# minaskar/pocomc

Measured on AMD Instinct MI355X. Metric: preconditioned MCMC steps/sec (1e4 particles, 32-D), higher is better.
Workload: dtype f32 flow (MFMA) + f64 step

## Files before the change

include/pocomc_amd.h:

```cpp
#ifndef POCOMC_AMD_H
#define POCOMC_AMD_H

#include <stdint.h>

#ifdef __cplusplus
extern "C" {
#endif

#define PMC_ABI_VERSION 9

const char* pmc_last_error(void);
int pmc_abi_version(void);
const char* pmc_build_id(void);


typedef struct pmc_maf {
    const float* packed;
    const int32_t* meta;
    int32_t D, H, T;
    int32_t Hp, Dp;
    int32_t nT, nXT, nOT;
    int64_t pk_per_transform;
    int32_t tri_ok;
    int32_t n_out;
// ... 366 lines not shown
    const pmc_prior_stage_t* prior_stage;
} pmc_step_ext_t;

int pmc_blob_rows_move(const int32_t* accept, const void* src, void* dst, int64_t n, int64_t row_bytes, void* stream);

#define PMC_ADAPT_TPCN 1
#define PMC_ADAPT_PRWM 2
#define PMC_ADAPT_RWM 3
#define PMC_ADAPT_MU 8

int pmc_rng_fill(const pmc_rng_t* rng, double gamma_shape, double* normal, double* gamma, double* uniform,
                 int64_t n, int32_t D, void* stream);
int pmc_event_synchronize(void* ev);

int pmc_propose_inverse(int kind, const float* cur32, const double* mu, const double* inv_cov, const double* chol,
                        double nu, double sigma, double cn_a, const pmc_rng_t* rng, double* prop64, double* quad,
                        double* quad_prop, const pmc_maf_t* maf, float* u_out, float* ladj, int64_t n, void* stream);

int pmc_step_pre(const pmc_step_t* s, const pmc_rng_t* rng, double nu, double sigma, double cn_a, void* stream);
int pmc_step_pre_deferred(const pmc_step_t* s, const pmc_rng_t* rng, double nu, double sigma, double cn_a, void* stream);
int pmc_step_fill_next(const pmc_step_t* s, const pmc_rng_t* rng, double nu, void* stream);
int pmc_step_handover(const pmc_step_t* s, int64_t step, int32_t epilogue, pmc_handover_t* out, int32_t* mode,
                      int32_t* clean_unknown);
int pmc_step_post(const pmc_step_t* s, const pmc_rng_t* rng, double beta, double nu, int want_mask,
                  int copy_sums, void* stream);
int pmc_step_lik_rows(const pmc_step_t* s, void* stream);
int pmc_step_prior_rows(const pmc_step_t* s, const void* logp, int logp_is_f32, void* stream);
int pmc_step_prior_stage(const pmc_step_t* s, void* stream);
int pmc_adapt_update(const double* const* parts, int32_t n_parts, int32_t D, double* total_out, double* h_sums,
                     double* adapt_state, int32_t adapt_mode, double c_sigma, double c_mu, double cap, double n_total,
                     const pmc_done_t* done, void* stream);
int pmc_stream_synchronize(void* stream);

void* pmc_comm_create(int32_t rank, int32_t world, int32_t width);
void* pmc_comm_create_host(int32_t rank, int32_t world, int32_t width);
int pmc_comm_kind(void* comm);
int pmc_comm_unlink(void* comm);
int pmc_comm_handle(void* comm, void* out64);
int pmc_comm_connect(void* comm, const void* handles);
void pmc_comm_destroy(void* comm);
int pmc_comm_adapt_update(void* comm, const double* const* parts, int32_t n_parts, int32_t D, double* total_out, double* h_sums,
                          double* adapt_state, int32_t adapt_mode, double c_sigma, double c_mu, double cap, double n_total,
                          const pmc_done_t* done, double timeout_s, void* stream);
int pmc_pipeline_set_comm(void* pipeline, void* comm);

void* pmc_pipeline_create(const pmc_step_t* const* lanes, int32_t n_lanes, uint64_t seed, const uint64_t* offsets,
                          void* prefetcher, double wait_timeout_s, void* stream);
void pmc_pipeline_destroy(void* pipeline);
int pmc_pipeline_start(void* pipeline, double nu, int64_t first_step);
int pmc_pipeline_next(void* pipeline, int32_t lane_done, double beta, double nu, int32_t adapt_mode, double c_sigma,
                      double c_mu, double cap, double n_total, int32_t more);
int pmc_pipeline_stats(void* pipeline, double* out, int32_t reset);
void* pmc_event_create(void);
int pmc_event_record(void* ev, void* stream);
float pmc_event_elapsed_ms(void* a, void* b);
void pmc_event_destroy(void* ev);


int pmc_logw(const double* logl, const double* beta, const double* logz, double beta_final,
             double* logw, int32_t T, int64_t N, void* stream);

int64_t pmc_reduce_workspace_bytes(int64_t P);
int pmc_logw_stats(const double* logw, int64_t P, int64_t k, double* stats, void* workspace, void* stream);

int64_t pmc_trim_workspace_bytes(int64_t P);
int pmc_trim_threshold(const double* w, int64_t P, double ess, int32_t bins, double* result,
                       void* workspace, int64_t workspace_bytes, void* stream);


int pmc_weights_from_logw(const double* logw, int64_t P, const double* stats, double* w, void* stream);

// ... 154 lines not shown
```

pocomc_amd/_lib.py:

```python
from __future__ import annotations

import ctypes as C
import os

_HERE = os.path.dirname(os.path.abspath(__file__))
LIB_PATH = os.environ.get("PMC_LIBRARY") or os.path.join(_HERE, "libpocomc_amd.so")

c_p = C.c_void_p


class pmc_maf_t(C.Structure):
    _fields_ = [("packed", c_p), ("meta", c_p),
                ("D", C.c_int32), ("H", C.c_int32), ("T", C.c_int32),
                ("Hp", C.c_int32), ("Dp", C.c_int32),
                ("nT", C.c_int32), ("nXT", C.c_int32), ("nOT", C.c_int32),
                ("pk_per_transform", C.c_int64),
                ("tri_ok", C.c_int32), ("n_out", C.c_int32),
                ("lane16", c_p), ("lane16_fmt", C.c_int32), ("reserved", C.c_int32)]


class pmc_inverse_plan_t(C.Structure):
    _fields_ = [(k, C.c_int32) for k in ("sweep", "fused", "epilogue", "maxo", "fm", "subsets", "waves", "helper_fmt",
                                         "lds_bytes")]

# ... 181 lines not shown
    "pmc_maf_valid_epoch": (C.c_int, [P(pmc_maf_t), c_p, c_p, c_p, i64, i64, c_p, c_p, c_p]),
    "pmc_neg_weighted_sum": (C.c_int, [c_p, c_p, c_p, C.c_float, c_p, i64, c_p]),
    "pmc_sum_f32": (C.c_int, [c_p, c_p, i64, c_p]),
    "pmc_adamw_step": (C.c_int, [c_p, c_p, c_p, c_p, i64, f64, f64, f64, f64, f64, f64, i64, c_p, c_p]),
    "pmc_scaler_inverse": (C.c_int, [P(pmc_scaler_t), c_p, c_p, c_p, c_p, c_p, c_p, c_p, i64, c_p]),
    "pmc_scaler_forward": (C.c_int, [P(pmc_scaler_t), c_p, c_p, i64, c_p]),
    "pmc_prior_logpdf": (C.c_int, [P(pmc_prior_t), c_p, c_p, c_p, i64, c_p]),
    "pmc_scaler_inverse_prior": (C.c_int, [P(pmc_scaler_t), P(pmc_prior_t), c_p, c_p, c_p, c_p, c_p, c_p, c_p, c_p,
                                           c_p, c_p, P(pmc_done_t), i64, c_p]),
    "pmc_wait_flag": (C.c_int, [c_p, i64, f64]),
    "pmc_propose": (C.c_int, [C.c_int, c_p, c_p, c_p, c_p, c_p, f64, f64, f64, P(pmc_rng_t),
                              c_p, c_p, c_p, c_p, i64, i32, c_p]),
    "pmc_accept_workspace_bytes": (i64, [i64, i32]),
    "pmc_accept": (C.c_int, [C.c_int, C.c_int, P(pmc_state_t), P(pmc_proposal_t), f64, f64,
                             P(pmc_rng_t), c_p, c_p, c_p, c_p, i64, i32, c_p]),
    "pmc_accept_armed": (C.c_int, [C.c_int, C.c_int, P(pmc_state_t), P(pmc_proposal_t), f64, f64,
                                   P(pmc_rng_t), c_p, c_p, c_p, c_p, P(pmc_done_t), c_p, i64, i32, c_p]),
    "pmc_propose_inverse": (C.c_int, [C.c_int, c_p, c_p, c_p, c_p, f64, f64, f64, P(pmc_rng_t), c_p, c_p, c_p,
                                      P(pmc_maf_t), c_p, c_p, i64, c_p]),
    "pmc_step_pre": (C.c_int, [P(pmc_step_t), P(pmc_rng_t), f64, f64, f64, c_p]),
    "pmc_step_pre_deferred": (C.c_int, [P(pmc_step_t), P(pmc_rng_t), f64, f64, f64, c_p]),
    "pmc_step_fill_next": (C.c_int, [P(pmc_step_t), P(pmc_rng_t), f64, c_p]),
    "pmc_step_handover": (C.c_int, [P(pmc_step_t), i64, i32, P(pmc_handover_t), P(i32), P(i32)]),
    "pmc_step_post": (C.c_int, [P(pmc_step_t), P(pmc_rng_t), f64, f64, C.c_int, C.c_int, c_p]),
    "pmc_step_lik_rows": (C.c_int, [P(pmc_step_t), c_p]),
    "pmc_step_prior_rows": (C.c_int, [P(pmc_step_t), c_p, C.c_int, c_p]),
    "pmc_step_prior_stage": (C.c_int, [P(pmc_step_t), c_p]),
    "pmc_blob_rows_move": (C.c_int, [c_p, c_p, c_p, i64, i64, c_p]),
    "pmc_stream_synchronize": (C.c_int, [c_p]),
    "pmc_pipeline_create": (C.c_void_p, [C.POINTER(C.c_void_p), i32, C.c_uint64, C.POINTER(C.c_uint64), c_p, f64, c_p]),
    "pmc_pipeline_set_comm": (C.c_int, [c_p, c_p]),
    "pmc_comm_create": (C.c_void_p, [i32, i32, i32]),
    "pmc_comm_create_host": (C.c_void_p, [i32, i32, i32]),
    "pmc_comm_kind": (C.c_int, [c_p]),
    "pmc_comm_unlink": (C.c_int, [c_p]),
    "pmc_comm_handle": (C.c_int, [c_p, c_p]),
    "pmc_comm_connect": (C.c_int, [c_p, c_p]),
    "pmc_comm_destroy": (None, [c_p]),
    "pmc_comm_adapt_update": (C.c_int, [c_p, C.POINTER(C.c_void_p), i32, i32, c_p, c_p, c_p, i32, f64, f64, f64, f64, P(pmc_done_t), f64,
                                        c_p]),
    "pmc_pipeline_destroy": (None, [c_p]),
    "pmc_pipeline_start": (C.c_int, [c_p, f64, i64]),
    "pmc_pipeline_next": (C.c_int, [c_p, i32, f64, f64, i32, f64, f64, f64, f64, i32]),
    "pmc_pipeline_stats": (C.c_int, [c_p, C.POINTER(C.c_double), i32]),
    "pmc_event_create": (c_p, []),
    "pmc_event_record": (C.c_int, [c_p, c_p]),
    "pmc_event_elapsed_ms": (C.c_float, [c_p, c_p]),
    "pmc_event_synchronize": (C.c_int, [c_p]),
    "pmc_weight_penalty": (C.c_int, [c_p, c_p, c_p, i64, f64, f64, C.c_float, c_p, c_p, c_p]),
    "pmc_add_noise_f32": (C.c_int, [c_p, i64, i32, C.c_float, C.c_uint64, C.c_uint64, c_p, c_p]),
    "pmc_add_noise_rows_f32": (C.c_int, [c_p, i64, i32, C.c_float, C.c_uint64, C.c_uint64, C.c_uint64, c_p, c_p]),
    "pmc_mean_distance_f32": (C.c_int, [c_p, i64, i32, i64, c_p, c_p]),
    "pmc_affine_rows": (C.c_int, [c_p, c_p, c_p, c_p, i64, i32, i32, c_p]),
    "pmc_sum_f64": (C.c_int, [c_p, i64, c_p, c_p]),
    "pmc_weights_from_logw": (C.c_int, [c_p, i64, c_p, c_p, c_p]),
    "pmc_trim_select_workspace_bytes": (C.c_int64, [i64]),
    "pmc_trim_select": (C.c_int, [c_p, i64, c_p, c_p, c_p, c_p, c_p, i64, c_p]),
    "pmc_moments_workspace_bytes": (C.c_int64, [i32]),
    "pmc_moments": (C.c_int, [c_p, c_p, c_p, c_p, i64, i32, c_p, c_p, c_p, c_p, i64, c_p]),
    "pmc_column_medians_workspace_bytes": (C.c_int64, [i64, i32, i32]),
    "pmc_column_medians": (C.c_int, [c_p, c_p, c_p, i64, i32, c_p, c_p, c_p, i64, c_p]),
    "pmc_student_em_workspace_bytes": (C.c_int64, [i64, i32]),
    "pmc_student_em": (C.c_int, [c_p, c_p, c_p, i64, i32, c_p, c_p, f64, i32, P(f64), c_p, i64, c_p]),
    "pmc_student_em_weighted_workspace_bytes": (C.c_int64, [i64, i32]),
# ... 107 lines not shown
```

pocomc_amd/csrc/scaler_body.h:

```cpp
#ifndef PMC_SCALER_BODY_H
#define PMC_SCALER_BODY_H

#include <hip/hip_runtime.h>
#include <math.h>
#include <stdint.h>
#include "../../include/pocomc_amd.h"

#pragma clang fp contract(off)

#define LOG_SQRT_2PI 0.91893853320467267
#define SQRT2 1.4142135623730951

__device__ __forceinline__ double np_pairwise_leaf(const double* a, int n) {
    if (n < 8) {
        double res = 0.0;
        for (int i = 0; i < n; ++i) res += a[i];
        return res;
    }
    double r0 = a[0], r1 = a[1], r2 = a[2], r3 = a[3], r4 = a[4], r5 = a[5], r6 = a[6], r7 = a[7];
    int i;
    for (i = 8; i < n - (n % 8); i += 8) {
        r0 += a[i + 0]; r1 += a[i + 1]; r2 += a[i + 2]; r3 += a[i + 3];
        r4 += a[i + 4]; r5 += a[i + 5]; r6 += a[i + 6]; r7 += a[i + 7];
    }
// ... 113 lines not shown
    const double z = (xv - f.loc) / f.pscale;
    return (-(z * z) / 2.0 - LOG_SQRT_2PI) - f.log_pscale;
}
template <class P>
__device__ __forceinline__ double prior_term(const P& pr, int j, double xv) {
    ScalerFeat f;
    f.loc = pr.loc[j]; f.pscale = pr.scale[j]; f.family = pr.family[j];
    f.log_pscale = log(f.pscale);
    return prior_term(f, xv);
}


__device__ __forceinline__ void scaler_element(const pmc_scaler_t& s, const ScalerFeat& f, double& u, double& x, double& J) {
    double t = s.scale ? f.mu + f.sigma * u : u;
    bound_inverse(f, s.logit, t, x, J);
    if (s.bc) {
        x = apply_bc(f, x);
        u = bound_forward(f, s.logit, s.scale, x);
        t = s.scale ? f.mu + f.sigma * u : u;
        bound_inverse(f, s.logit, t, x, J);
    }
}

__device__ __forceinline__ void handover_complete(const pmc_handover_t& h, long long* stamps, int tid) {
    if (!h.done_flag) return;
    __builtin_amdgcn_fence(__ATOMIC_RELEASE, "agent");
    __syncthreads();
    if (stamps && tid == 0) stamps[blockIdx.x * 8 + 5] = wall_clock64();
    if (tid == 0) {
        const unsigned t = __hip_atomic_fetch_add(h.done_ticket, 1u, __ATOMIC_ACQ_REL, __HIP_MEMORY_SCOPE_AGENT);
        if (t == gridDim.x - 1) {
            *h.done_ticket = 0u;
            if (h.bad_count && h.bad_flag) {
                const unsigned bad = __hip_atomic_exchange(h.bad_count, 0u, __ATOMIC_ACQ_REL, __HIP_MEMORY_SCOPE_AGENT);
                *h.bad_flag = (long long)bad;
            }
            __threadfence_system();
            __hip_atomic_store(h.done_flag, (int64_t)h.done_value, __ATOMIC_RELEASE, __HIP_MEMORY_SCOPE_SYSTEM);
        }
    }
}

struct ScalerEpi {
    int on, have_prior;
    pmc_scaler_t s;
    pmc_prior_un_t pr;
    double* u_out; double* x_out; double* ldj_out; int32_t* finite_out; double* logp_out;
    pmc_handover_t h;
    long long* stamps;
};

static inline size_t scaler_epilogue_lds_bytes(int D) {
    return (size_t)(2 * 16 * D + D * 17) * sizeof(double) + 16 * sizeof(int);
}

__device__ __forceinline__ void scaler_epilogue_rows(const ScalerEpi& e, const double* Jt, const double* Pt, const double* Xt,
                                                     int* rowfin, int64_t row0, int64_t n, int D, int tid, int nthr) {
    const pmc_scaler_t& s = e.s;
    const pmc_handover_t& h = e.h;
    const int rows = (int)min((int64_t)16, n - row0);
    const int n8 = D - (D % 8);
    for (int rb = 0; rb < 16; rb += nthr >> 3) {
        const int r = rb + (tid >> 3), i = tid & 7;
        const bool live = r < rows;
        const double* a = Jt + (size_t)r * D;
        double acc = 0.0;
        if (live && D >= 8) {
// ... 8 lines not shown
                const double p0 = P[j], p1 = P[j + 1], p2 = P[j + 2], p3 = P[j + 3];
                const double p4 = P[j + 4], p5 = P[j + 5], p6 = P[j + 6], p7 = P[j + 7];
                lps += p0; lps += p1; lps += p2; lps += p3; lps += p4; lps += p5; lps += p6; lps += p7;
            }
            for (; j < D; ++j) lps += P[j];
        }
        acc = acc + __shfl_xor(acc, 1, 8);
        acc = acc + __shfl_xor(acc, 2, 8);
        acc = acc + __shfl_xor(acc, 4, 8);
        lps = __shfl(lps, 4, 8);
        if (live && i == 0) {
            double l;
            if (D < 8) {
                l = 0.0;
                for (int k = 0; k < D; ++k) l += a[k];
            } else {
                l = acc;
                for (int k = n8; k < D; ++k) l += a[k];
            }
            if (s.scale) l = s.sum_log_sigma + l;
            e.ldj_out[row0 + r] = l;
            const int fin = (rowfin[r] && isfinite(l)) ? 1 : 0;
            e.finite_out[row0 + r] = fin;
            if (h.finite_copy) h.finite_copy[row0 + r] = fin;
            bool clean = fin != 0;
            if (e.have_prior) {
                const double lp = fin ? lps : -INFINITY;
                e.logp_out[row0 + r] = lp;
                if (h.logp_copy) h.logp_copy[row0 + r] = lp;
                clean = clean && isfinite(lp);
            }
            if (h.bad_count && !clean) atomicAdd(h.bad_count, 1u);
            if (h.fill_x) rowfin[r] = clean ? 1 : 0;
        }
    }
    if (h.fill_x) __syncthreads();
    if (e.stamps && tid == 0) e.stamps[blockIdx.x * 8 + 2] = wall_clock64();
    if (e.stamps && tid == 0) e.stamps[blockIdx.x * 8 + 3] = wall_clock64();
    if (h.x_colmajor) {
        const int dj = nthr / rows, dr = nthr - dj * rows;
        int j = tid / rows, r = tid - j * rows;
        for (int el = tid; el < rows * D; el += nthr) {
            h.x_colmajor[(size_t)j * n + row0 + r] = (h.fill_x && !rowfin[r]) ? h.fill_x[(row0 + r) * D + j] : Xt[j * 17 + r];
            j += dj; r += dr;
            if (r >= rows) { r -= rows; ++j; }
        }
    }
    if (e.stamps && tid == 0) e.stamps[blockIdx.x * 8 + 4] = wall_clock64();
    handover_complete(h, e.stamps, tid);
}

template <class LIDX>
__device__ __forceinline__ void scaler_epilogue(const ScalerEpi& e, const float* X, const int* __restrict__ rof,
                                                double* scr, int64_t row0, int64_t n, int D, int tid, int nthr,
                                                LIDX lidx_of) {
    double* Jt = scr;
    double* Pt = Jt + 16 * D;
    double* Xt = Pt + 16 * D;
    int* rowfin = reinterpret_cast<int*>(Xt + D * 17);
    const int rows = (int)min((int64_t)16, n - row0);
    if (tid < 16) rowfin[tid] = 1;
    if (e.stamps && tid == 0) e.stamps[blockIdx.x * 8 + 0] = wall_clock64();
    const int rpp = nthr / D;
    const int r0 = tid / D, j = tid - r0 * D;
    const bool act = r0 < rpp;
    ScalerFeat f;
    int rk = 0;
    if (act) {
        scaler_feat_request(f, e.s, e.have_prior ? &e.pr : nullptr, j);
        rk = rof[j];
    }
    __syncthreads();
// ... 21 lines not shown
```

pocomc_amd/csrc/step.hip:

```cpp

#include <hip/hip_runtime.h>
#include <stdio.h>
#include <time.h>
#include "pmc_internal.h"
#include "propose_body.h"
#include "blob_move.h"
#include "flow_prior_body.h"

#ifdef PMC_DEBUG_HOOKS
static long long* g_epilogue_stamps = nullptr;
static int64_t g_epilogue_stamps_n = 0;
static bool g_stage_per_lane = false;
#endif

static bool step_prefills(const pmc_step_t* s, const pmc_rng_t* rng) {
    return s->rng_ready && s->rng_normal[0] && s->rng_normal[1] && s->rng_uniform[0] && s->rng_uniform[1] &&
           (s->kind != PMC_KIND_TPCN || (s->rng_gamma[0] && s->rng_gamma[1])) && !rng->normal && !rng->gamma && !rng->uniform;
}

extern "C" int pmc_step_fill_next(const pmc_step_t* s, const pmc_rng_t* rng, double nu, void* stream) {
    if (!s || !rng) return pmc_fail("pmc_step_fill_next: null argument");
    if (!step_prefills(s, rng)) return 0;
    const int rb = (int)(rng->step & 1);
    const double gshape = (s->kind == PMC_KIND_TPCN) ? 0.5 * ((double)s->D + nu) : 0.0;
// ... 8 lines not shown
static const pmc_prior_stage_t* step_stage(const pmc_step_t* s) {
    return (s->ext == PMC_STEP_EXT || s->ext == PMC_STEP_EXT2) ? reinterpret_cast<const pmc_step_ext_t*>(s)->prior_stage : nullptr;
}
static const pmc_prior_blocks_stage_t* step_blocks_stage(const pmc_step_t* s) {
    return s->ext == PMC_STEP_EXT2 ? reinterpret_cast<const pmc_step_ext2_t*>(s)->blocks_stage : nullptr;
}
static bool step_has_stage(const pmc_step_t* s) { return step_stage(s) || step_blocks_stage(s); }
static pmc_step_ext2_t step_copy(const pmc_step_t* s) {
    pmc_step_ext2_t c{};
    c.step = *s;
    c.prior_stage = step_stage(s);
    c.blocks_stage = step_blocks_stage(s);
    return c;
}

static bool step_direct(const pmc_step_t* s) { return s->host_direct && !s->p_xT; }

static bool step_devlik(const pmc_step_t* s) { return s->lik_x && (s->prior || s->prior_rows); }

static int step_mode(const pmc_step_t* s, bool devlik) {
    return devlik ? PMC_HANDOVER_DEVLIK : step_direct(s) ? PMC_HANDOVER_DIRECT : PMC_HANDOVER_COPIES;
}

static void step_handover(const pmc_step_t* s, int64_t step, bool epilogue, pmc_handover_t* h, int32_t* mode,
                          int32_t* clean_unknown) {
    const bool devlik = step_devlik(s);
    *mode = step_mode(s, devlik);
    const bool host = *mode == PMC_HANDOVER_DIRECT;
    *h = pmc_handover_t{};
    h->x_colmajor = devlik ? s->lik_x : step_direct(s) ? s->h_x : s->p_xT;
    if (host) {
        h->finite_copy = s->h_fin;
        if (s->prior) h->logp_copy = s->h_logp_out;
    }
    const bool done = host && s->h_done && s->done_ticket;
    if (done) { h->done_ticket = s->done_ticket; h->done_flag = s->h_done; h->done_value = step + 1; }
    const bool word = done && s->h_clean && s->clean_count;
    if (word && (epilogue || (h->x_colmajor && s->prior))) {
        h->bad_count = s->clean_count;
        h->bad_flag = s->h_clean;
        if (s->fill_rejected && h->x_colmajor) h->fill_x = s->cur.x;
    }
    if (devlik) { h->bad_count = s->clean_count; h->bad_flag = nullptr; h->fill_x = s->cur.x; }
    *clean_unknown = s->h_clean && !(word && h->x_colmajor && (epilogue || s->prior));
}

extern "C" int pmc_step_handover(const pmc_step_t* s, int64_t step, int32_t epilogue, pmc_handover_t* out, int32_t* mode,
                                 int32_t* clean_unknown) {
    if (!s || !out || !mode || !clean_unknown) return pmc_fail("pmc_step_handover: null argument");
    step_handover(s, step, epilogue != 0, out, mode, clean_unknown);
    return 0;
}

template <bool JOINT>
__global__ __launch_bounds__(256) void prior_stage_close_kernel(const float* __restrict__ lp32, const double* __restrict__ ldj,
                                                                const double* __restrict__ rest_logp,
                                                                const int32_t* __restrict__ inside,
                                                                const int32_t* __restrict__ fin, double* __restrict__ logp,
                                                                unsigned long long* __restrict__ count,
                                                                long long* __restrict__ h_count, int64_t n) {
    __shared__ unsigned wave_bad[4];
    const int tid = threadIdx.x;
    const int64_t r = (int64_t)blockIdx.x * 256 + tid;
    bool bad = false;
    if (r < n) {
        double v = -INFINITY;
        if (fin[r]) {
            v = JOINT ? joint_prior_join(lp32[r], ldj[r], rest_logp[r], inside[r]) : flow_prior_join(lp32[r], ldj[r], inside[r]);
            bad = !isfinite(v);
        }
        logp[r] = v;
    }
    const unsigned nb = (unsigned)__popcll(__ballot(bad));
// ... 137 lines not shown
    int rc = joint ? pmc_joint_prior_pre(g->scaler, g->flow_cols, g->rest, g->rest_cols, s->p_x, s->D, 1, n, g->u32, g->ldj,
                                         g->rest_logp, g->inside, stream)
                   : pmc_flow_prior_pre(g->scaler, s->p_x, s->D, 1, n, g->u32, g->ldj, g->inside, stream);
    if (rc) return rc;
    rc = g->image16 ? pmc_maf_forward_bf16(g->maf, g->image16, g->image_per_transform, g->u32, g->z, nullptr, g->lp32, n, nullptr, stream)
                    : pmc_maf_forward(g->maf, g->u32, g->z, nullptr, g->lp32, n, stream);
    if (rc) return rc;
    const dim3 grid((unsigned)((n + 255) / 256));
    if (joint)
        hipLaunchKernelGGL(prior_stage_close_kernel<true>, grid, dim3(256), 0, (hipStream_t)stream, g->lp32, g->ldj, g->rest_logp,
                           g->inside, s->p_fin, s->p_logp, g->count, (long long*)g->h_count, n);
    else
        hipLaunchKernelGGL(prior_stage_close_kernel<false>, grid, dim3(256), 0, (hipStream_t)stream, g->lp32, g->ldj,
                           (const double*)nullptr, g->inside, s->p_fin, s->p_logp, g->count, (long long*)g->h_count, n);
    return pmc_check_launch("prior_stage_close_kernel");
}

extern "C" int pmc_step_prior_stage(const pmc_step_t* s, void* stream) {
    if (int e = prior_stage_check(s)) return e;
    return prior_stage_enqueue(s, stream);
}

static int step_pre(const pmc_step_t* s, const pmc_rng_t* rng, double nu, double sigma, double cn_a, void* stream,
                    bool fill_next) {
    if (!s || !rng) return pmc_fail("pmc_step_pre: null argument");
    if (step_has_stage(s)) { if (int e = prior_stage_check(s)) return e; }
    hipStream_t st = (hipStream_t)stream;
    const int64_t n = s->n;
    const int32_t D = s->D;
    const bool tpcn = (s->kind == PMC_KIND_TPCN);
    pmc_rng_t rr = *rng;
    const bool prefill = step_prefills(s, rng);
    const pmc_rng_t* rng_in = rng;
    const int rb = (int)(rng->step & 1);
    const double gshape = tpcn ? 0.5 * ((double)D + nu) : 0.0;
    if (prefill) {
        if (*s->rng_ready != (int64_t)rng->step) {
            int rcf = pmc_rng_fill(rng, gshape, s->rng_normal[rb], s->rng_gamma[rb], s->rng_uniform[rb], n, D, stream);
            if (rcf) return rcf;
        }
        rr.normal = s->rng_normal[rb];
        rr.gamma = tpcn ? s->rng_gamma[rb] : nullptr;
        rng = &rr;
    }
    auto finish = [&]() -> int {
        if (s->ev_pre_done) (void)hipEventRecord((hipEvent_t)s->ev_pre_done, st);
        if (step_has_stage(s) && fill_next) { if (int e = prior_stage_enqueue(s, stream)) return e; }
        if (prefill && fill_next) return pmc_step_fill_next(s, rng_in, nu, stream);
        return 0;
    };
    const double* mu = s->mu;
    const double* adapt = (s->adapt_state && s->adapt_mode) ? s->adapt_state : nullptr;
    if (!adapt && tpcn && s->h_mu) {
        if (step_direct(s)) mu = s->h_mu;
        else if (hipMemcpyAsync((void*)s->mu, s->h_mu, (size_t)D * sizeof(double), hipMemcpyHostToDevice, st) != hipSuccess)
            return pmc_fail("pmc_step_pre: H2D mu");
    }
    int rc;
    const pmc_prior_t* pr = s->prior;
    double* lp = pr ? s->p_logp : nullptr;
    if (step_devlik(s) && !s->clean_count) return pmc_fail("pmc_step_pre: a device likelihood needs clean_count");
    const bool want_epi = s->preconditioned && !(s->no_fuse & 3) && s->scaler && s->scaler->low && s->scaler->high &&
                          s->scaler->kind && s->scaler->log_width && (!s->scaler->scale || (s->scaler->mu && s->scaler->sigma)) &&
                          (!pr || (pr->family && pr->loc && pr->scale && pr->D == D && pr->n_extended == 0));
    pmc_inverse_plan_t plan{};
    if (s->preconditioned && !(s->no_fuse & 1)) {
        rc = pmc_plan_inverse(s->maf, n, s->inverse_algo, PMC_FUSED_STEP, want_epi, want_epi ? s->scaler->D : 0, &plan);
        if (rc) return rc;
    }
    pmc_handover_t hand;
    int32_t mode, clean_unknown;
    step_handover(s, (int64_t)rng->step, plan.epilogue != 0, &hand, &mode, &clean_unknown);
    if (clean_unknown) *s->h_clean = -1;
    if (plan.sweep != PMC_SWEEP_NONE) {
        ProposeArgs pa{s->kind, s->cur.theta32, mu, s->inv_cov, s->chol, nu, sigma, cn_a, *rng, s->p_theta64,
                       tpcn ? s->quad : nullptr, tpcn ? s->p_quad : nullptr, adapt};
        if (plan.epilogue) {
            ScalerEpi& epi = pa.epi;
            epi.on = 1;
            epi.s = *s->scaler;
            epi.have_prior = pr ? 1 : 0;
            if (pr) epi.pr = pmc_prior_un_t{pr->family, pr->loc, pr->scale, pr->D, pr->reserved};
            epi.u_out = s->p_u; epi.x_out = s->p_x; epi.ldj_out = s->p_logdetj; epi.finite_out = s->p_fin; epi.logp_out = lp;
            epi.h = hand;
#ifdef PMC_DEBUG_HOOKS
            epi.stamps = (n == g_epilogue_stamps_n) ? g_epilogue_stamps : nullptr;
#endif
        }
        if (s->ev_inv0) (void)hipEventRecord((hipEvent_t)s->ev_inv0, st);
        rc = pmc_launch_inverse(&plan, &pa, s->maf, nullptr, s->p_u32, s->p_ldjf, n, st);
        if (rc) return rc;
        if (s->ev_inv1) (void)hipEventRecord((hipEvent_t)s->ev_inv1, st);
    } else {
        rc = pmc_propose_adapt(s->kind, s->preconditioned ? s->cur.theta32 : nullptr,
                               s->preconditioned ? nullptr : s->cur.u, mu, s->inv_cov, s->chol, nu, sigma, cn_a, rng,
                               s->p_theta64, s->preconditioned ? s->p_theta32 : nullptr, tpcn ? s->quad : nullptr,
                               tpcn ? s->p_quad : nullptr, n, D, stream, adapt);
        if (rc) return rc;
        if (s->preconditioned) {
            if (s->ev_inv0) (void)hipEventRecord((hipEvent_t)s->ev_inv0, st);
            rc = pmc_maf_inverse(s->maf, s->p_theta32, s->p_u32, s->p_ldjf, n, s->inverse_algo, stream);
            if (s->ev_inv1) (void)hipEventRecord((hipEvent_t)s->ev_inv1, st);
            if (rc) return rc;
        }
    }
    if (!plan.epilogue) {
        rc = pmc_scaler_inverse_prior_ex(s->scaler, pr, s->preconditioned ? s->p_u32 : nullptr,
// ... 244 lines not shown
}

extern "C" int pmc_event_synchronize(void* ev) {
    hipError_t e = hipEventSynchronize((hipEvent_t)ev);
    return e == hipSuccess ? 0 : pmc_fail_hip(e, "hipEventSynchronize");
}
extern "C" float pmc_event_elapsed_ms(void* a, void* b) {
    float ms = -1.0f;
    if (hipEventElapsedTime(&ms, (hipEvent_t)a, (hipEvent_t)b) != hipSuccess) return -1.0f;
    return ms;
}
extern "C" void pmc_event_destroy(void* ev) { if (ev) (void)hipEventDestroy((hipEvent_t)ev); }


struct pmc_pipeline {
    int n_lanes;
    const pmc_step_t* lanes[8];
    pmc_rng_t rng[8];
    int64_t step;
    void* stream;
    void* prefetcher;
    void* comm;
    double timeout;
    double t_wait_x, t_wait_sums, t_enq_accept, t_enq_pre;
    int64_t n_steps;
};

static double now_s() {
    struct timespec t;
    clock_gettime(CLOCK_MONOTONIC, &t);
    return (double)t.tv_sec + 1e-9 * (double)t.tv_nsec;
}

extern "C" void* pmc_pipeline_create(const pmc_step_t* const* lanes, int32_t n_lanes, uint64_t seed,
                                     const uint64_t* offsets, void* prefetcher, double wait_timeout_s, void* stream) {
    if (!lanes || n_lanes < 1 || n_lanes > 8 || !offsets) { pmc_fail("pmc_pipeline_create: 1..8 lanes"); return nullptr; }
    for (int k = 0; k < n_lanes; ++k) {
        const pmc_step_t* s = lanes[k];
        if (!s || !s->host_direct || !s->h_done || !s->done_ticket || !s->adapt_state || s->p_xT) {
            pmc_fail("pmc_pipeline_create: every lane needs host_direct buffers, completion words and adapt_state");
            return nullptr;
        }
        if (s->adapt_state != lanes[0]->adapt_state) { pmc_fail("pmc_pipeline_create: one adapt_state for all lanes"); return nullptr; }
    }
    pmc_pipeline* p = new pmc_pipeline();
    p->n_lanes = n_lanes;
    for (int k = 0; k < n_lanes; ++k) {
        p->lanes[k] = lanes[k];
        p->rng[k] = pmc_rng_t{nullptr, nullptr, nullptr, seed, 0, offsets[k]};
    }
    p->step = 0;
    p->stream = stream;
    p->prefetcher = prefetcher;
    p->comm = nullptr;
    p->timeout = wait_timeout_s;
    p->t_wait_x = p->t_wait_sums = p->t_enq_accept = p->t_enq_pre = 0.0;
    p->n_steps = 0;
    return p;
}

extern "C" void pmc_pipeline_destroy(void* pp) { delete (pmc_pipeline*)pp; }

extern "C" int pmc_pipeline_set_comm(void* pp, void* comm) {
    pmc_pipeline* p = (pmc_pipeline*)pp;
    if (!p) return pmc_fail("pmc_pipeline_set_comm: null pipeline");
    p->comm = comm;
    return 0;
}

static int pipeline_enqueue_pre(pmc_pipeline* p, int64_t step, double nu) {
#ifdef PMC_DEBUG_HOOKS
    const bool stage_per_lane = g_stage_per_lane;
#else
    const bool stage_per_lane = false;
#endif
    for (int k = 0; k < p->n_lanes; ++k) {
        pmc_step_ext2_t sx = step_copy(p->lanes[k]);
        pmc_step_t& s = sx.step;
        s.adapt_mode = 1;
        p->rng[k].step = (uint64_t)step;
        const int rc = step_pre(&s, &p->rng[k], nu, 0.0, 0.0, p->stream, false);
        if (rc) return rc;
        if (step_has_stage(&s) && stage_per_lane) { if (int e = prior_stage_enqueue(&s, p->stream)) return e; }
        if (p->prefetcher)
            (void)pmc_prefetcher_submit(p->prefetcher, s.h_done, step + 1, s.h_x, (int64_t)s.n * s.D * 8, p->timeout > 0 ? p->timeout : 1.0);
    }
    for (int k = 0; k < p->n_lanes; ++k) {
        if (!step_has_stage(p->lanes[k]) || stage_per_lane) continue;
        const int rc = prior_stage_enqueue(p->lanes[k], p->stream);
        if (rc) return rc;
    }
    for (int k = 0; k < p->n_lanes; ++k) {
        const int rc = pmc_step_fill_next(p->lanes[k], &p->rng[k], nu, p->stream);
        if (rc) return rc;
    }
    return 0;
}

extern "C" int pmc_pipeline_start(void* pp, double nu, int64_t first_step) {
    pmc_pipeline* p = (pmc_pipeline*)pp;
    if (!p) return pmc_fail("pmc_pipeline_start: null pipeline");
    p->step = first_step;
    return pipeline_enqueue_pre(p, first_step, nu);
}
// ... 67 lines not shown
```

pocomc_amd/mcmc.py:

```python
from __future__ import annotations

import ctypes as C
import os
import time
from functools import partial

import numpy as np
import torch
import torch.distributed as dist

from . import _lib

KINDS = ("preconditioned_pcn", "preconditioned_rwm", "pcn", "rwm")
PMC_KIND_TPCN, PMC_KIND_RWM = 0, 1


def _env_wait_timeout(): return float(os.environ.get("PMC_WAIT_TIMEOUT", "600"))
def _env_no_fuse(): return int(os.environ.get("PMC_NO_FUSE", "0"))
def _env_c_pipeline(): return os.environ.get("PMC_C_PIPELINE", "1") != "0"
def _env_c_allreduce(): return os.environ.get("PMC_C_ALLREDUCE", "1") != "0"
def _env_comm_mailbox(): return os.environ.get("PMC_COMM_MAILBOX", "")


PMC_ADAPT_TPCN, PMC_ADAPT_PRWM, PMC_ADAPT_RWM, PMC_ADAPT_MU = 1, 2, 3, 8
# ... 403 lines not shown
        for b in range(2):
            self._step.rng_normal[b] = self._pf_normal[b].data_ptr()
            self._step.rng_gamma[b] = self._pf_gamma[b].data_ptr()
            self._step.rng_uniform[b] = self._pf_uniform[b].data_ptr()
        self._step.ev_pre_done = self._ev_pre
        self.spin_wait = True
        self.h_done = pin(2, dt=torch.int64)
        self.h_done.zero_()
        self._done_ticket = torch.zeros(1, dtype=torch.int32, device=dev)
        self.h_clean = pin(1, dt=torch.int64)
        self.h_clean.fill_(-1)
        self._np_clean = self.h_clean.numpy()
        self._clean_count = torch.zeros(1, dtype=torch.int32, device=dev)
        self.fill_rejected = True
        self.fill_rejected_max = 0.05
        self._direct_now = False
        self._pre_cfg = None
        self.adapt_state = f64(D + 2)
        self._h_adapt = pin(D + 2)
        self.device_adapt = False
        self.prior_desc = None
        self.host_direct = (x_order == "F")
        self.step_idx = 0
        self.host_threads = 1
        self.host_cores = None
        self.prefetcher = None
        self._pool = None
        self.stream = None
        self.events = None
        self.host_timers = None
        self.wait_timeout = _wait_timeout(None)
        self.device_likelihood = False
        self.p_xl = None
        self.h_calls = None
        self.blobs = None
        self.p_blobs = None
        self.h_blobs = None
        self._np_blobs = None
        self.device_logprior = False
        self._stage = None
        self._stage_read = 0
        self._sums_part = None

    def __del__(self):
        if getattr(self, "_recycle", False):
            for t in getattr(self, "_pins", ()):
# ... 134 lines not shown
                self.r_gamma.copy_(torch.from_numpy(np.ascontiguousarray(replay["gamma"], dtype=np.float64)))
            self.r_normal.copy_(torch.from_numpy(np.ascontiguousarray(replay["z"], dtype=np.float64)))
            self.r_uniform.copy_(torch.from_numpy(np.ascontiguousarray(replay["u"], dtype=np.float64)))
            return _lib.pmc_rng_t(gamma=self.r_gamma.data_ptr() if self.tpcn else None,
                                  normal=self.r_normal.data_ptr(), uniform=self.r_uniform.data_ptr(),
                                  seed=0, step=self.step_idx, offset=self.offset)
        return _lib.pmc_rng_t(gamma=None, normal=None, uniform=None, seed=self.seed, step=self.step_idx,
                              offset=self.offset)

    def can_pipeline(self):
        return bool(not self._instrumented() and self.host_direct and self.x_order == "F"
                    and self.spin_wait and self.D <= 256)

    def adapt_upload(self, sigma, mu=None):
        a = self._h_adapt.numpy()
        a[0] = sigma
        a[1] = (1.0 - sigma ** 2.0) ** 0.5 if self.tpcn else 0.0
        a[2:] = 0.0 if mu is None else mu
        self.adapt_state.copy_(self._h_adapt, non_blocking=True)
        self._step.adapt_state = self.adapt_state.data_ptr()
        self.device_adapt = True

    def propose(self, sigma, nu=0.0, replay=None, step=None, defer_fill=False):
        if self._instrumented():
            return self._propose_instrumented(sigma, nu, replay)
        if replay is not None:
            self._rng_cur = self._rng(replay)
        else:
            self._rng_fast.step = self.step_idx if step is None else int(step)
            self._rng_cur = self._rng_fast
        self._step.adapt_mode = 1 if self.device_adapt else 0
        self._configure_step()
        if self.device_adapt:
            sigma, cn_a = 0.0, 0.0
        else:
            cn_a = float((1.0 - sigma ** 2.0) ** 0.5) if self.tpcn else 0.0
        self._stream = self.stream.cuda_stream if self.stream is not None else _lib.stream_handle()
        pre = self.lib.pmc_step_pre_deferred if defer_fill else self.lib.pmc_step_pre
        _lib.check(pre(C.byref(self._step), C.byref(self._rng_cur), float(nu), float(sigma), cn_a, self._stream), "pmc_step_pre")
        if self.prefetcher is not None and self._direct_now:
            self.lib.pmc_prefetcher_submit(self.prefetcher, self.h_done.data_ptr(), int(self._rng_cur.step) + 1,
                                           self.h_x.data_ptr(), self.n * self.D * 8, self.wait_timeout)

    def fill_next(self, nu=0.0):
        if self._instrumented():
            return
# ... 58 lines not shown
    def _wait_pre_step(self):
        if self._instrumented():
            torch.cuda.current_stream().synchronize()
        elif self._direct_now:
            _lib.check(self.lib.pmc_wait_flag(self.h_done.data_ptr(), self.step_idx + 1, self.wait_timeout), "pmc_wait_flag")
        else:
            _lib.check(self.lib.pmc_event_synchronize(self._ev_pre), "pmc_event_synchronize")

    def evaluate(self, log_prior, log_like, have_blobs=False, blobs=None, waited=False):
        tm = self.host_timers
        t0 = time.perf_counter() if tm is not None else 0.0
        if not waited:
            self._wait_pre_step()
        if self.prior_desc is not None or self._stage is not None:
            log_prior = None
        if tm is not None:
            tm["wait_device"] += time.perf_counter() - t0
            log_prior = None if log_prior is None else _timed(log_prior, tm, "prior")
            log_like = _timed(log_like, tm, "likelihood")
        n = self.n
        x_prime, logp_prime, logl_prime, fin_i = self._np_x, self._np_logp, self._np_logl, self._np_fin
        bad = -1
        if ((waited or not self._instrumented()) and self._direct_now and self.prior_desc is not None
                and self.host_threads <= 1 and not have_blobs):
            bad = int(self._np_clean[0])
        keep = self._np_blobs is not None
        if bad == 0:
            out = log_like(x_prime)
            logl_prime[:] = self._keep_blobs(out, slice(None), n) if keep else out[0]
            return n, None
        all_fin = fin_i.all()
        if all_fin and self.host_threads > 1 and not have_blobs:
            return self._evaluate_threaded(log_prior, log_like), None
        fin = None if all_fin else fin_i.astype(bool)
        if log_prior is not None:
            if all_fin:
                logp_prime[:] = log_prior(x_prime)
            else:
                logp_prime[fin] = log_prior(x_prime[fin])
                logp_prime[~fin] = -np.inf
        if self._stage is not None:
            mask = np.ones(n, dtype=bool) if all_fin else fin
        else:
            mask = np.isfinite(logp_prime) if all_fin else fin & np.isfinite(logp_prime)
        whole = bool(mask.all())
        block = whole or (self._step.fill_rejected and 0 < bad <= self.fill_rejected_max * n)
        xs, rows = (x_prime, slice(None)) if block else (x_prime[mask], mask)
# ... 172 lines not shown
        self.lanes = []
        for k, (lo, hi) in enumerate(self.bounds):
            if streams:
                st = torch.cuda.Stream(device=self.device, priority=-1 if k == 0 else 0)
                with torch.cuda.stream(st):
                    e = StepEngine(kind, hi - lo, n_dim, flow, scaler, group=group,
                                   shard_offset=int(shard_offset) + lo, seed=seed, x_order=x_order)
                e.stream = st
            else:
                e = StepEngine(kind, hi - lo, n_dim, flow, scaler, group=group, shard_offset=int(shard_offset) + lo,
                               seed=seed, x_order=x_order)
            self.lanes.append(e)
        self.lib = self.lanes[0].lib
        self.tpcn, self.pre = self.lanes[0].tpcn, self.lanes[0].pre
        self._tot = torch.zeros(self.D + 4, dtype=torch.float64, device=self.device)
        self._h_tot = torch.zeros(self.D + 4, dtype=torch.float64).pin_memory()
        self._ev = [torch.cuda.Event() for _ in self.lanes]
        self.host_timers = None
        self._h_flag = torch.zeros(1, dtype=torch.int64).pin_memory()
        self._flag_value = 0
        self._tot_part = (C.c_void_p * 1)(self._tot.data_ptr())
        self.c_pipeline = _env_c_pipeline()
        self._pipe = None

    def __del__(self):
        self._drop_pipe()

    def _drop_pipe(self):
        if getattr(self, "_pipe", None):
            try:
                self.lib.pmc_pipeline_destroy(self._pipe)
            except Exception:
                pass
            self._pipe = None

    def _each(self, fn):
        out = []
        for e in self.lanes:
            if e.stream is None:
                out.append(fn(e))
            else:
                with torch.cuda.stream(e.stream):
                    out.append(fn(e))
        return out

    def configure(self, **kw):
# ... 19 lines not shown

    def start_pipeline(self, sigma, mu, nu):
        first = self.lanes[0]
        first.adapt_upload(sigma, mu)
        for e in self.lanes[1:]:
            e._step.adapt_state = first.adapt_state.data_ptr()
            e.device_adapt = True
        sharded = _sharded(self.group)
        self._drop_pipe()
        comm = small_comm(self.lib, self.group, self.D + 4) if (sharded and self.c_pipeline) else None
        if self.c_pipeline and (not sharded or comm) and len(self.lanes) <= 8:
            K = len(self.lanes)
            for e in self.lanes:
                e._configure_step()
            assert all(e._direct_now for e in self.lanes)
            self._lane_structs = (C.c_void_p * K)(*[C.addressof(e._step) for e in self.lanes])
            offs = (C.c_uint64 * K)(*[e.offset for e in self.lanes])
            stream = first.stream.cuda_stream if first.stream is not None else _lib.stream_handle()
            first._stream = stream
            self._pipe = self.lib.pmc_pipeline_create(self._lane_structs, K, first.seed, offs, first.prefetcher,
                                                      float(first.wait_timeout), stream)
            if not self._pipe:
                _lib.check(1, "pmc_pipeline_create")
            if comm:
                _lib.check(self.lib.pmc_pipeline_set_comm(self._pipe, comm), "pmc_pipeline_set_comm")
            _lib.check(self.lib.pmc_pipeline_start(self._pipe, float(nu), int(first.step_idx)), "pmc_pipeline_start")
            return
        self._propose_lanes(nu)

    def _propose_lanes(self, nu, ahead=0):
        for e in self.lanes:
            e.host_timers = self.host_timers
            e.propose(None, nu, step=e.step_idx + ahead, defer_fill=True)
        for e in self.lanes:
            e.stage_enqueue()
        for e in self.lanes:
            e.fill_next(nu)

    def resume_pipeline(self, nu):
        first = self.lanes[0]
        if self._pipe:
            _lib.check(self.lib.pmc_pipeline_start(self._pipe, float(nu), int(first.step_idx)), "pmc_pipeline_start")
            return
        self._propose_lanes(nu)

    def pipeline_stats(self, reset=True):
        if not self._pipe:
            return None
        out = (C.c_double * 6)()
        _lib.check(self.lib.pmc_pipeline_stats(self._pipe, out, int(reset)), "pmc_pipeline_stats")
        return dict(wait_x=out[0], wait_sums=out[1], enqueue_accept=out[2], enqueue_next_pre=out[3], steps=int(out[4]))

    def step_pipelined(self, beta, nu, coefficients, n_total, log_prior, log_like, more=True):
        if self._pipe:
            nxt, P = self.lib.pmc_pipeline_next, self._pipe
            mode, c_sigma, c_mu, cap = coefficients
            tm = self.host_timers
            if nxt(P, -1, beta, nu, mode, c_sigma, c_mu, cap, n_total, 0):
                _lib.check(1, "pmc_pipeline_next")
            calls = 0
            for k, e in enumerate(self.lanes):
                e.host_timers = tm
                calls += e.evaluate(log_prior, log_like, waited=True)[0]
                if nxt(P, k, beta, nu, mode, c_sigma, c_mu, cap, n_total, int(more)):
                    _lib.check(1, "pmc_pipeline_next")
            for e in self.lanes:
                e.step_idx += 1
            sums = self.lanes[-1]._np_sums
            if sums[0] != sums[0]:
                raise _lib.PocomcAmdError("sharded step: a rank did not deliver its sums within wait_timeout")
            return calls, sums
        sharded = _sharded(self.group)
        lib, D = self.lib, self.D
        tm = self.host_timers
        clock = time.perf_counter
        calls = 0
        last = self.lanes[-1]
        for e in self.lanes:
            e.host_timers = tm
            calls += e.evaluate(log_prior, log_like)[0]
            t0 = clock() if tm is not None else 0.0
            if e is last and not sharded:
                e.accept_enqueue(beta, nu, host_sums=True, adapt=coefficients, n_total=n_total, others=self.lanes[:-1])
            elif e is last:
                if e._step.h_sums != self._tot.data_ptr():
                    e._step.h_sums = self._tot.data_ptr()
                e.accept_enqueue(beta, nu, host_sums=True, others=self.lanes[:-1])
            else:
# ... 396 lines not shown
```

Before: 3300.

## Write host handover masks only when the epilogue finds bad rows

Adds a masks-on-demand mode to the fused scaler epilogue. Per-row writes of the finite/logp copies into host-visible handover buffers are skipped, and the last block copies the masks only when the bad-row count is nonzero. It also drops a redundant system fence before the done flag store. This cuts host-memory traffic on clean steps in exchange for a serialized copy by one block when bad rows occur, plus more Python-side state tracking.

```diff
diff --git a/include/pocomc_amd.h b/include/pocomc_amd.h
--- a/include/pocomc_amd.h
+++ b/include/pocomc_amd.h
@@ -412,6 +412,8 @@
 int pmc_step_fill_next(const pmc_step_t* s, const pmc_rng_t* rng, double nu, void* stream);
 int pmc_step_handover(const pmc_step_t* s, int64_t step, int32_t epilogue, pmc_handover_t* out, int32_t* mode,
                       int32_t* clean_unknown);
+int pmc_step_handover_ex(const pmc_step_t* s, int64_t step, int32_t epilogue, int32_t ask, pmc_handover_t* out,
+                         int32_t* mode, int32_t* clean_unknown, int32_t* masks_on_demand);
 int pmc_step_post(const pmc_step_t* s, const pmc_rng_t* rng, double beta, double nu, int want_mask,
                   int copy_sums, void* stream);
 int pmc_step_lik_rows(const pmc_step_t* s, void* stream);
@@ -437,6 +439,7 @@
 void* pmc_pipeline_create(const pmc_step_t* const* lanes, int32_t n_lanes, uint64_t seed, const uint64_t* offsets,
                           void* prefetcher, double wait_timeout_s, void* stream);
 void pmc_pipeline_destroy(void* pipeline);
+int pmc_pipeline_set_masks_on_demand(void* pipeline, int32_t on);
 int pmc_pipeline_start(void* pipeline, double nu, int64_t first_step);
 int pmc_pipeline_next(void* pipeline, int32_t lane_done, double beta, double nu, int32_t adapt_mode, double c_sigma,
                       double c_mu, double cap, double n_total, int32_t more);
diff --git a/pocomc_amd/_lib.py b/pocomc_amd/_lib.py
--- a/pocomc_amd/_lib.py
+++ b/pocomc_amd/_lib.py
@@ -227,6 +227,7 @@
     "pmc_step_pre_deferred": (C.c_int, [P(pmc_step_t), P(pmc_rng_t), f64, f64, f64, c_p]),
     "pmc_step_fill_next": (C.c_int, [P(pmc_step_t), P(pmc_rng_t), f64, c_p]),
     "pmc_step_handover": (C.c_int, [P(pmc_step_t), i64, i32, P(pmc_handover_t), P(i32), P(i32)]),
+    "pmc_step_handover_ex": (C.c_int, [P(pmc_step_t), i64, i32, i32, P(pmc_handover_t), P(i32), P(i32), P(i32)]),
     "pmc_step_post": (C.c_int, [P(pmc_step_t), P(pmc_rng_t), f64, f64, C.c_int, C.c_int, c_p]),
     "pmc_step_lik_rows": (C.c_int, [P(pmc_step_t), c_p]),
     "pmc_step_prior_rows": (C.c_int, [P(pmc_step_t), c_p, C.c_int, c_p]),
@@ -245,6 +246,7 @@
     "pmc_comm_adapt_update": (C.c_int, [c_p, C.POINTER(C.c_void_p), i32, i32, c_p, c_p, c_p, i32, f64, f64, f64, f64, P(pmc_done_t), f64,
                                         c_p]),
     "pmc_pipeline_destroy": (None, [c_p]),
+    "pmc_pipeline_set_masks_on_demand": (C.c_int, [c_p, i32]),
     "pmc_pipeline_start": (C.c_int, [c_p, f64, i64]),
     "pmc_pipeline_next": (C.c_int, [c_p, i32, f64, f64, i32, f64, f64, f64, f64, i32]),
     "pmc_pipeline_stats": (C.c_int, [c_p, C.POINTER(C.c_double), i32]),
diff --git a/pocomc_amd/csrc/scaler_body.h b/pocomc_amd/csrc/scaler_body.h
--- a/pocomc_amd/csrc/scaler_body.h
+++ b/pocomc_amd/csrc/scaler_body.h
@@ -159,11 +159,65 @@
     }
 }
 
-__device__ __forceinline__ void handover_complete(const pmc_handover_t& h, long long* stamps, int tid) {
+__device__ __forceinline__ void handover_masks(const pmc_handover_t& h, const int32_t* fin_src, const double* lp_src,
+                                               int64_t n, int tid, int nthr) {
+    for (int64_t i0 = tid; i0 < n; i0 += (int64_t)nthr * 4) {
+        int32_t f[4] = {0, 0, 0, 0};
+        double l[4] = {0.0, 0.0, 0.0, 0.0};
+#pragma unroll
+        for (int k = 0; k < 4; ++k) {
+            const int64_t i = i0 + (int64_t)k * nthr;
+            if (i < n) {
+                f[k] = fin_src[i];
+                if (lp_src) l[k] = lp_src[i];
+            }
+        }
+#pragma unroll
+        for (int k = 0; k < 4; ++k) {
+            const int64_t i = i0 + (int64_t)k * nthr;
+            if (i < n) {
+                h.finite_copy[i] = f[k];
+                if (lp_src) h.logp_copy[i] = l[k];
+            }
+        }
+    }
+}
+
+__device__ __forceinline__ void handover_complete(const pmc_handover_t& h, long long* stamps, int tid, int nthr = 0,
+                                                  int64_t n = 0, int* word2 = nullptr, const int32_t* fin_src = nullptr,
+                                                  const double* lp_src = nullptr) {
     if (!h.done_flag) return;
     __builtin_amdgcn_fence(__ATOMIC_RELEASE, "agent");
     __syncthreads();
     if (stamps && tid == 0) stamps[blockIdx.x * 8 + 5] = wall_clock64();
+    if (word2) {
+        if (tid == 0) {
+            const unsigned t = __hip_atomic_fetch_add(h.done_ticket, 1u, __ATOMIC_ACQ_REL, __HIP_MEMORY_SCOPE_AGENT);
+            const int last = t == gridDim.x - 1;
+            unsigned bad = 0u;
+            if (last) {
+                *h.done_ticket = 0u;
+                bad = __hip_atomic_exchange(h.bad_count, 0u, __ATOMIC_ACQ_REL, __HIP_MEMORY_SCOPE_AGENT);
+            }
+            word2[0] = last;
+            word2[1] = (int)bad;
+        }
+        __syncthreads();
+        if (word2[0]) {
+            const unsigned bad = (unsigned)word2[1];
+            if (bad > 0u) {
+                __builtin_amdgcn_fence(__ATOMIC_ACQUIRE, "agent");
+                handover_masks(h, fin_src, (lp_src && h.logp_copy) ? lp_src : nullptr, n, tid, nthr);
+                __builtin_amdgcn_fence(__ATOMIC_RELEASE, "agent");
+                __syncthreads();
+            }
+            if (tid == 0) {
+                *h.bad_flag = (long long)bad;
+                __hip_atomic_store(h.done_flag, (int64_t)h.done_value, __ATOMIC_RELEASE, __HIP_MEMORY_SCOPE_SYSTEM);
+            }
+        }
+        return;
+    }
     if (tid == 0) {
         const unsigned t = __hip_atomic_fetch_add(h.done_ticket, 1u, __ATOMIC_ACQ_REL, __HIP_MEMORY_SCOPE_AGENT);
         if (t == gridDim.x - 1) {
@@ -172,7 +226,6 @@
                 const unsigned bad = __hip_atomic_exchange(h.bad_count, 0u, __ATOMIC_ACQ_REL, __HIP_MEMORY_SCOPE_AGENT);
                 *h.bad_flag = (long long)bad;
             }
-            __threadfence_system();
             __hip_atomic_store(h.done_flag, (int64_t)h.done_value, __ATOMIC_RELEASE, __HIP_MEMORY_SCOPE_SYSTEM);
         }
     }
@@ -180,6 +233,7 @@
 
 struct ScalerEpi {
     int on, have_prior;
+    int masks_on_demand;
     pmc_scaler_t s;
     pmc_prior_un_t pr;
     double* u_out; double* x_out; double* ldj_out; int32_t* finite_out; double* logp_out;
@@ -234,12 +288,12 @@
             e.ldj_out[row0 + r] = l;
             const int fin = (rowfin[r] && isfinite(l)) ? 1 : 0;
             e.finite_out[row0 + r] = fin;
-            if (h.finite_copy) h.finite_copy[row0 + r] = fin;
+            if (h.finite_copy && !e.masks_on_demand) h.finite_copy[row0 + r] = fin;
             bool clean = fin != 0;
             if (e.have_prior) {
                 const double lp = fin ? lps : -INFINITY;
                 e.logp_out[row0 + r] = lp;
-                if (h.logp_copy) h.logp_copy[row0 + r] = lp;
+                if (h.logp_copy && !e.masks_on_demand) h.logp_copy[row0 + r] = lp;
                 clean = clean && isfinite(lp);
             }
             if (h.bad_count && !clean) atomicAdd(h.bad_count, 1u);
@@ -259,7 +313,8 @@
         }
     }
     if (e.stamps && tid == 0) e.stamps[blockIdx.x * 8 + 4] = wall_clock64();
-    handover_complete(h, e.stamps, tid);
+    handover_complete(h, e.stamps, tid, nthr, n, e.masks_on_demand ? rowfin : nullptr, e.finite_out,
+                      e.have_prior ? e.logp_out : nullptr);
 }
 
 template <class LIDX>
diff --git a/pocomc_amd/csrc/step.hip b/pocomc_amd/csrc/step.hip
--- a/pocomc_amd/csrc/step.hip
+++ b/pocomc_amd/csrc/step.hip
@@ -54,8 +54,8 @@
     return devlik ? PMC_HANDOVER_DEVLIK : step_direct(s) ? PMC_HANDOVER_DIRECT : PMC_HANDOVER_COPIES;
 }
 
-static void step_handover(const pmc_step_t* s, int64_t step, bool epilogue, pmc_handover_t* h, int32_t* mode,
-                          int32_t* clean_unknown) {
+static void step_handover(const pmc_step_t* s, int64_t step, bool epilogue, bool ask_on_demand, pmc_handover_t* h,
+                          int32_t* mode, int32_t* clean_unknown, int32_t* on_demand) {
     const bool devlik = step_devlik(s);
     *mode = step_mode(s, devlik);
     const bool host = *mode == PMC_HANDOVER_DIRECT;
@@ -74,13 +74,22 @@
         if (s->fill_rejected && h->x_colmajor) h->fill_x = s->cur.x;
     }
     if (devlik) { h->bad_count = s->clean_count; h->bad_flag = nullptr; h->fill_x = s->cur.x; }
+    *on_demand = (ask_on_demand && epilogue && h->done_flag && h->bad_count && h->bad_flag) ? 1 : 0;
     *clean_unknown = s->h_clean && !(word && h->x_colmajor && (epilogue || s->prior));
 }
 
 extern "C" int pmc_step_handover(const pmc_step_t* s, int64_t step, int32_t epilogue, pmc_handover_t* out, int32_t* mode,
                                  int32_t* clean_unknown) {
     if (!s || !out || !mode || !clean_unknown) return pmc_fail("pmc_step_handover: null argument");
-    step_handover(s, step, epilogue != 0, out, mode, clean_unknown);
+    int32_t on_demand;
+    step_handover(s, step, epilogue != 0, false, out, mode, clean_unknown, &on_demand);
+    return 0;
+}
+
+extern "C" int pmc_step_handover_ex(const pmc_step_t* s, int64_t step, int32_t epilogue, int32_t ask, pmc_handover_t* out,
+                                    int32_t* mode, int32_t* clean_unknown, int32_t* masks_on_demand) {
+    if (!s || !out || !mode || !clean_unknown || !masks_on_demand) return pmc_fail("pmc_step_handover_ex: null argument");
+    step_handover(s, step, epilogue != 0, ask != 0, out, mode, clean_unknown, masks_on_demand);
     return 0;
 }
 
@@ -264,7 +273,7 @@
 }
 
 static int step_pre(const pmc_step_t* s, const pmc_rng_t* rng, double nu, double sigma, double cn_a, void* stream,
-                    bool fill_next) {
+                    bool fill_next, bool masks_on_demand = false) {
     if (!s || !rng) return pmc_fail("pmc_step_pre: null argument");
     if (step_has_stage(s)) { if (int e = prior_stage_check(s)) return e; }
     hipStream_t st = (hipStream_t)stream;
@@ -311,8 +320,8 @@
         if (rc) return rc;
     }
     pmc_handover_t hand;
-    int32_t mode, clean_unknown;
-    step_handover(s, (int64_t)rng->step, plan.epilogue != 0, &hand, &mode, &clean_unknown);
+    int32_t mode, clean_unknown, on_demand;
+    step_handover(s, (int64_t)rng->step, plan.epilogue != 0, masks_on_demand, &hand, &mode, &clean_unknown, &on_demand);
     if (clean_unknown) *s->h_clean = -1;
     if (plan.sweep != PMC_SWEEP_NONE) {
         ProposeArgs pa{s->kind, s->cur.theta32, mu, s->inv_cov, s->chol, nu, sigma, cn_a, *rng, s->p_theta64,
@@ -325,6 +334,7 @@
             if (pr) epi.pr = pmc_prior_un_t{pr->family, pr->loc, pr->scale, pr->D, pr->reserved};
             epi.u_out = s->p_u; epi.x_out = s->p_x; epi.ldj_out = s->p_logdetj; epi.finite_out = s->p_fin; epi.logp_out = lp;
             epi.h = hand;
+            epi.masks_on_demand = on_demand;
 #ifdef PMC_DEBUG_HOOKS
             epi.stamps = (n == g_epilogue_stamps_n) ? g_epilogue_stamps : nullptr;
 #endif
@@ -615,6 +625,7 @@
     void* prefetcher;
     void* comm;
     double timeout;
+    bool masks_on_demand;
     double t_wait_x, t_wait_sums, t_enq_accept, t_enq_pre;
     int64_t n_steps;
 };
@@ -647,6 +658,7 @@
     p->prefetcher = prefetcher;
     p->comm = nullptr;
     p->timeout = wait_timeout_s;
+    p->masks_on_demand = false;
     p->t_wait_x = p->t_wait_sums = p->t_enq_accept = p->t_enq_pre = 0.0;
     p->n_steps = 0;
     return p;
@@ -658,6 +670,13 @@
     pmc_pipeline* p = (pmc_pipeline*)pp;
     if (!p) return pmc_fail("pmc_pipeline_set_comm: null pipeline");
     p->comm = comm;
+    return 0;
+}
+
+extern "C" int pmc_pipeline_set_masks_on_demand(void* pp, int32_t on) {
+    pmc_pipeline* p = (pmc_pipeline*)pp;
+    if (!p) return pmc_fail("pmc_pipeline_set_masks_on_demand: null pipeline");
+    p->masks_on_demand = on != 0;
     return 0;
 }
 
@@ -672,7 +691,7 @@
         pmc_step_t& s = sx.step;
         s.adapt_mode = 1;
         p->rng[k].step = (uint64_t)step;
-        const int rc = step_pre(&s, &p->rng[k], nu, 0.0, 0.0, p->stream, false);
+        const int rc = step_pre(&s, &p->rng[k], nu, 0.0, 0.0, p->stream, false, p->masks_on_demand);
         if (rc) return rc;
         if (step_has_stage(&s) && stage_per_lane) { if (int e = prior_stage_enqueue(&s, p->stream)) return e; }
         if (p->prefetcher)
diff --git a/pocomc_amd/mcmc.py b/pocomc_amd/mcmc.py
--- a/pocomc_amd/mcmc.py
+++ b/pocomc_amd/mcmc.py
@@ -449,6 +449,7 @@
         self.prior_desc = None
         self.host_direct = (x_order == "F")
         self.step_idx = 0
+        self.masks_on_demand = False
         self.host_threads = 1
         self.host_cores = None
         self.prefetcher = None
@@ -629,6 +630,7 @@
         self.device_adapt = True
 
     def propose(self, sigma, nu=0.0, replay=None, step=None, defer_fill=False):
+        self.masks_on_demand = False
         if self._instrumented():
             return self._propose_instrumented(sigma, nu, replay)
         if replay is not None:
@@ -733,7 +735,7 @@
         x_prime, logp_prime, logl_prime, fin_i = self._np_x, self._np_logp, self._np_logl, self._np_fin
         bad = -1
         if ((waited or not self._instrumented()) and self._direct_now and self.prior_desc is not None
-                and self.host_threads <= 1 and not have_blobs):
+                and (self.host_threads <= 1 or self.masks_on_demand) and not have_blobs):
             bad = int(self._np_clean[0])
         keep = self._np_blobs is not None
         if bad == 0:
@@ -952,6 +954,8 @@
         self._tot_part = (C.c_void_p * 1)(self._tot.data_ptr())
         self.c_pipeline = _env_c_pipeline()
         self._pipe = None
+        self.masks_on_demand = True
+        self._masks_set = False
 
     def __del__(self):
         self._drop_pipe()
@@ -1017,11 +1021,25 @@
                                                       float(first.wait_timeout), stream)
             if not self._pipe:
                 _lib.check(1, "pmc_pipeline_create")
+            self._masks_set = False
+            self._sync_masks_on_demand()
             if comm:
                 _lib.check(self.lib.pmc_pipeline_set_comm(self._pipe, comm), "pmc_pipeline_set_comm")
             _lib.check(self.lib.pmc_pipeline_start(self._pipe, float(nu), int(first.step_idx)), "pmc_pipeline_start")
+            self._masks_enqueued()
             return
         self._propose_lanes(nu)
+
+    def _sync_masks_on_demand(self):
+        want = self.masks_on_demand and all(e._direct_now and e.prior_desc is not None and e.host_threads <= 1
+                                            for e in self.lanes)
+        if want != self._masks_set:
+            _lib.check(self.lib.pmc_pipeline_set_masks_on_demand(self._pipe, int(want)), "pmc_pipeline_set_masks_on_demand")
+            self._masks_set = want
+
+    def _masks_enqueued(self):
+        for e in self.lanes:
+            e.masks_on_demand = self._masks_set
 
     def _propose_lanes(self, nu, ahead=0):
         for e in self.lanes:
@@ -1035,7 +1053,9 @@
     def resume_pipeline(self, nu):
         first = self.lanes[0]
         if self._pipe:
+            self._sync_masks_on_demand()
             _lib.check(self.lib.pmc_pipeline_start(self._pipe, float(nu), int(first.step_idx)), "pmc_pipeline_start")
+            self._masks_enqueued()
             return
         self._propose_lanes(nu)
 
@@ -1054,11 +1074,14 @@
             if nxt(P, -1, beta, nu, mode, c_sigma, c_mu, cap, n_total, 0):
                 _lib.check(1, "pmc_pipeline_next")
             calls = 0
+            self._sync_masks_on_demand()
             for k, e in enumerate(self.lanes):
                 e.host_timers = tm
                 calls += e.evaluate(log_prior, log_like, waited=True)[0]
                 if nxt(P, k, beta, nu, mode, c_sigma, c_mu, cap, n_total, int(more)):
                     _lib.check(1, "pmc_pipeline_next")
+            if more:
+                self._masks_enqueued()
             for e in self.lanes:
                 e.step_idx += 1
             sums = self.lanes[-1]._np_sums
```

After: 3111. -5.7%, worse.
